# CIAM-Group/ComputerVision_Codes

Measured on AMD Instinct MI355X. Metric: frames/sec spatial-extract + per-video TCN latency, Cholec80, 1/2/4/8 GPU, higher is better.
Workload: dtype bf16

## Files before the change

### computervision_codes_amd/_lib.py

```python
from __future__ import annotations

import ctypes as C
import os

import torch

_HERE = os.path.dirname(os.path.abspath(__file__))
LIB_PATH = os.path.join(_HERE, "libmt4hip.so")

MT4_F32 = 0
MT4_BF16 = 1


class ConvDesc(C.Structure):
    _fields_ = [
        ("x", C.c_void_p), ("w", C.c_void_p), ("bias", C.c_void_p), ("residual", C.c_void_p), ("y", C.c_void_p),
        ("out_row_map", C.c_void_p),
        ("B", C.c_int32), ("H", C.c_int32), ("W", C.c_int32), ("Cin", C.c_int32),
        ("Ho", C.c_int32), ("Wo", C.c_int32), ("Cout", C.c_int32),
        ("KH", C.c_int32), ("KW", C.c_int32),
        ("stride_h", C.c_int32), ("stride_w", C.c_int32),
        ("pad_h", C.c_int32), ("pad_w", C.c_int32),
        ("dil_h", C.c_int32), ("dil_w", C.c_int32),
        ("relu", C.c_int32), ("dtype", C.c_int32), ("out_dtype", C.c_int32), ("tile", C.c_int32),
# ... 73 lines not shown
    "mt4_bn_stats_t": (C.c_int, [_vp, _i32, _vp, _vp, _vp, _vp, _vp, C.c_int64, _i32, C.c_float, C.c_float, _vp]),
    "mt4_avgpool1d_rows": (C.c_int, [_vp, _vp, _i32, _i32, _i32, _i32, _i32, _i32, _vp]),
    "mt4_interp_linear_rows": (C.c_int, [_vp, _vp, _i32, _i32, _i32, _i32, _i32, _vp]),
    "mt4_avgpool1d_rows_bwd_f32": (C.c_int, [_vp, _vp, _i32, _i32, _i32, _i32, _i32, _vp]),
    "mt4_interp_linear_rows_bwd_f32": (C.c_int, [_vp, _vp, _i32, _i32, _i32, _i32, _vp]),
    "mt4_bn_apply_sums_f32": (C.c_int, [_vp] * 10 + [C.c_int64, _i32, C.c_float, C.c_float, _i32, _vp]),
    "mt4_bn_apply_sums_t": (C.c_int, [_vp, _i32] + [_vp] * 9 + [C.c_int64, _i32, C.c_float, C.c_float, _i32, _vp]),
    "mt4_bn_apply_t": (C.c_int, [_vp, _i32, _vp, _vp, _vp, _vp, _vp, _vp, C.c_int64, _i32, _i32, _vp]),
    "mt4_bn_backward_t": (C.c_int, [_vp, _vp, _vp, _i32] + [_vp] * 9 + [C.c_int64, _i32, _i32, _vp]),
    "mt4_wgrad_conv2d_bf16": (C.c_int, [_vp, _vp, _vp] + [_i32] * 9 + [_vp]),
    "mt4_maxpool3x3s2_bwd_bf16": (C.c_int, [_vp, _vp, _vp, _i32, _i32, _i32, _i32, _vp]),
    "mt4_avgpool_bwd_bf16": (C.c_int, [_vp, _vp, _i32, _i32, _i32, _vp]),
    "mt4_cast_f32_bf16": (C.c_int, [_vp, _vp, C.c_int64, _vp]),
    "mt4_refresh_weights": (C.c_int, [_vp, _i32, C.c_int64, _vp]),
    "mt4_repack_weight_bf16": (C.c_int, [_vp, _vp, _i32, _i32, _i32, _i32, _vp]),
    "mt4_kd_mix_bwd_f32": (C.c_int, [_vp] * 9 + [_i32, _i32, _vp]),
    "mt4_tcn_conv": (C.c_int, [C.POINTER(TcnDesc), _vp]),
    "mt4_tcn_dilated_residual_layer": (C.c_int, [_vp] * 7 + [_i32] * 5 + [_vp]),
    "mt4_tcn_stage": (C.c_int, [_vp] * 5 + [C.POINTER(_vp)] * 4 + [_i32] * 5 + [_vp]),
    "mt4_bottleneck_packed_bytes": (C.c_int64, [_i32, _i32]),
    "mt4_bottleneck_pack_bf16": (C.c_int, [_vp] * 4 + [_i32, _vp, _vp]),
    "mt4_bottleneck_fused_bf16": (C.c_int, [_vp] * 7 + [_i32] * 5 + [_vp]),
    "mt4_pack_fragments_bf16": (C.c_int, [_vp, _i32, _i32, _vp, _vp]),
    "mt4_chain_gemm_bf16": (C.c_int, [_vp, C.c_int64, C.c_int64, _i32, _vp, _vp, _i32, _vp, _vp, _i32, _vp, _vp, _i32, _vp, _i32, _vp, _vp]),
    "mt4_bottleneck_next_packed_bytes": (C.c_int64, []),
    "mt4_bottleneck_pack_next_bf16": (C.c_int, [_vp, _vp, _vp]),
    "mt4_bottleneck_fused_next_bf16": (C.c_int, [_vp, _vp, _vp, _vp, _vp, _vp, _vp, _vp, _vp, _i32, _i32, _i32, _vp]),
    "mt4_fpn_topdown": (C.c_int, [_vp, _vp, _i32, C.c_int64, _i32, _vp]),
    "mt4_tcn_layer_fused_bf16": (C.c_int, [_vp, _vp, _vp, _vp, _vp, _vp, _i32, _i32, _i32, _i32, _vp]),
    "mt4_tcn_linear_ln_f32": (C.c_int, [_vp, _vp, _vp, _vp, _vp, _vp, _i32, _i32, _i32, C.c_float, _i32, _vp, _vp, _vp]),
    "mt4_tcn_linear_stats_f32": (C.c_int, [_vp, _vp, _vp, _vp, _vp, _i32, _i32, _i32, _i32, _vp, _vp]),
    "mt4_bgemm_f32": (C.c_int, [_vp, _vp, _vp, _i32, _i32, _i32, _i32, _i32, C.POINTER(C.c_int64), C.POINTER(C.c_int64), C.POINTER(C.c_int64),
                                C.c_float, _i32, _vp]),
    "mt4_softmax_rows_f32": (C.c_int, [_vp, C.c_int64, _i32, C.c_float, _vp]),
    "mt4_softmax_bwd_rows_f32": (C.c_int, [_vp, _vp, C.c_int64, _i32, C.c_float, _vp]),
    "mt4_layernorm_bwd_f32": (C.c_int, [_vp, _vp, _vp, _vp, _vp, _vp, C.c_int64, _i32, C.c_float, _i32, _vp]),
    "mt4_gelu_f32": (C.c_int, [_vp, _vp, C.c_int64, _vp]),
    "mt4_gelu_bwd_f32": (C.c_int, [_vp, _vp, _vp, C.c_int64, _vp]),
    "mt4_dwconv1d_k3_bwd_f32": (C.c_int, [_vp, _vp, _vp, _vp, _vp, _vp, _i32, _i32, _i32, _vp]),
    "mt4_gather_rows_f32": (C.c_int, [_vp, _vp, _vp, C.c_int64, _i32, _i32, _i32, _i32, _i32, _vp]),
    "mt4_add_bias_mask_f32": (C.c_int, [_vp, _vp, _vp, _vp, C.c_int64, _i32, _i32, _i32, _vp]),
    "mt4_relpos_table_grad_f32": (C.c_int, [_vp, _vp, _vp, C.c_int64, _i32, _i32, _vp]),
    "mt4_rowscale_add_f32": (C.c_int, [_vp, _vp, _vp, _vp, C.c_int64, _i32, _i32, _vp]),
    "mt4_groupwise_linear_bwd_f32": (C.c_int, [_vp] * 6 + [_i32, _i32, _i32, _vp]),
    "mt4_sum_over_batch_f32": (C.c_int, [_vp, _vp, _i32, C.c_int64, _i32, _vp]),
    "mt4_dropout_mask_f32": (C.c_int, [_vp, C.c_int64, C.c_int64, C.c_int64, C.c_float, _vp]),
    "mt4_axpby_f32": (C.c_int, [_vp, _vp, C.c_int64, C.c_float, C.c_float, _vp]),
# ... 49 lines not shown
```

### computervision_codes_amd/csrc/chain_gemm.hip

```cpp
#include "mt4_common.h"

typedef __bf16 bf16x8_t __attribute__((ext_vector_type(8)));

namespace {

struct ChainK {
    const char* x;
    long long x_ld_bytes;
    const char* w1f;
    const float* b1;
    const char* r1;
    char* y1;
    const char* w2f;
    const float* b2;
    const char* r2;
    char* y2;
    int M, K1, N1, N2, act1, act2;
};

constexpr int BM = 128;
constexpr int CH = 128;
constexpr int PLANE = BM * 128;

__device__ __forceinline__ void act4(float (&v)[4], int a) {
    if (a == 1) {
#pragma unroll
        for (int e = 0; e < 4; ++e) v[e] = fmaxf(v[e], 0.f);
    } else if (a == 2) {
        gelu_erf_n(v);
    }
}

template <int NT2, int NKS1, bool CONV, int NCHUNK>
__global__ __launch_bounds__(512, 2) void chain_gemm_kernel(const ChainK a) {
    extern __shared__ __attribute__((aligned(16))) char smem[];
    const int tid = threadIdx.x, lane = tid & 63;
    const int wave = __builtin_amdgcn_readfirstlane(tid >> 6);
    const int r16 = lane & 15, q = lane >> 4;
    const int m0 = blockIdx.x * BM;
    constexpr int nks1 = NKS1;
    constexpr int ACT1 = CONV ? 1 : 2;
    constexpr int nchunk = NCHUNK;
    const int mlast = a.M - 1;
    char* const Xs = smem;
    char* const Hb = smem + nks1 * PLANE;
    float* const B1s = (float*)(Hb + 4 * PLANE);
    const long long n1b = (long long)a.N1 * 2, n2b = (long long)a.N2 * 2;

    {
        uint4 xv[NKS1 * 2];
#pragma unroll
        for (int i = 0; i < NKS1 * 2; ++i) {
            const int pid = tid + i * 512;
            const int plane = pid >> 10, row = (pid >> 3) & 127, ck = pid & 7;
            xv[i] = *(const uint4*)(a.x + (long long)min(m0 + row, mlast) * a.x_ld_bytes + plane * 128 + ck * 16);
        }
#pragma unroll
        for (int i = 0; i < NKS1 * 2; ++i) {
            const int pid = tid + i * 512;
            const int plane = pid >> 10, row = (pid >> 3) & 127, ck = pid & 7;
            *(uint4*)(Xs + plane * PLANE + row * 128 + ((ck ^ (row & 7)) << 4)) = xv[i];
        }
    }
    struct R4 { uint4 v0, v1, v2, v3; };
    R4 rr;
    auto load_r = [&](int c) __attribute__((always_inline)) -> R4 {
        R4 r;
        const char* base = a.r1 + (long long)(c * CH) * 2;
        auto piece = [&](int i) __attribute__((always_inline)) -> uint4 {
            const int pid = tid + i * 512;
            const int plane = pid >> 10, row = (pid >> 3) & 127, ck = pid & 7;
            return *(const uint4*)(base + (long long)min(m0 + row, mlast) * n1b + plane * 128 + ck * 16);
        };
        r.v0 = piece(0); r.v1 = piece(1); r.v2 = piece(2); r.v3 = piece(3);
        return r;
    };
    auto put_r = [&](int c, const R4& r) __attribute__((always_inline)) {
        char* hb = Hb + (c & 1) * (2 * PLANE);
        auto dst = [&](int i) __attribute__((always_inline)) -> uint4* {
            const int pid = tid + i * 512;
            const int plane = pid >> 10, row = (pid >> 3) & 127, ck = pid & 7;
            return (uint4*)(hb + plane * PLANE + row * 128 + ((ck ^ (row & 7)) << 4));
        };
        *dst(0) = r.v0; *dst(1) = r.v1; *dst(2) = r.v2; *dst(3) = r.v3;
    };
    for (int i = tid; i < nchunk * (CH / 4); i += 512) *(float4*)(B1s + i * 4) = *(const float4*)(a.b1 + i * 4);
    if constexpr (CONV) {
        put_r(0, load_r(0));
        rr = load_r(min(1, nchunk - 1));
    }

    const int f1_stride = (a.K1 >> 5) * 1024;
    const int f2_stride = (a.N1 >> 5) * 1024;
    const char* const w1p = a.w1f + (long long)wave * f1_stride + lane * 16;
    const char* const w2p = a.w2f + (long long)(wave * NT2) * f2_stride + lane * 16;
    uint4 fa1[2 * NKS1];
    auto load_w1 = [&](int c) __attribute__((always_inline)) {
        const char* p = w1p + (long long)c * 8 * f1_stride;
#pragma unroll
        for (int s = 0; s < 2 * NKS1; ++s) fa1[s] = *(const uint4*)(p + s * 1024);
    };
    load_w1(0);

    f32x4 acc2[NT2][8];
#pragma unroll
    for (int t = 0; t < NT2; ++t) {
        const float4 b = *(const float4*)(a.b2 + (wave * NT2 + t) * 16 + q * 4);
#pragma unroll
        for (int j = 0; j < 8; ++j) acc2[t][j] = (f32x4){b.x, b.y, b.z, b.w};
    }
    __syncthreads();

    const int frag_off = r16 * 128;
    const int sw0 = ((0 * 4 + q) ^ (r16 & 7)) << 4, sw1 = ((1 * 4 + q) ^ (r16 & 7)) << 4;

#pragma unroll
    for (int c = 0; c < nchunk; ++c) {
        char* const hb = Hb + (c & 1) * (2 * PLANE);
        f32x4 acc1[8];
        {
            const float4 b = *(const float4*)(B1s + (c * 8 + wave) * 16 + q * 4);
#pragma unroll
            for (int j = 0; j < 8; ++j) acc1[j] = (f32x4){b.x, b.y, b.z, b.w};
        }
        uint4 fa2[NT2][4];
#pragma unroll
        for (int ks = 0; ks < NKS1; ++ks) {
            const char* xp = Xs + ks * PLANE + frag_off;
#pragma unroll
            for (int kk = 0; kk < 2; ++kk) {
                const bf16x8_t A = __builtin_bit_cast(bf16x8_t, fa1[ks * 2 + kk]);
#pragma unroll
                for (int jh = 0; jh < 8; jh += 4) {
                    uint4 bx[4];
#pragma unroll
                    for (int j = 0; j < 4; ++j) bx[j] = *(const uint4*)(xp + (jh + j) * (16 * 128) + (kk ? sw1 : sw0));
#pragma unroll
                    for (int j = 0; j < 4; ++j)
                        acc1[jh + j] = __builtin_amdgcn_mfma_f32_16x16x32_bf16(A, __builtin_bit_cast(bf16x8_t, bx[j]), acc1[jh + j], 0, 0, 0);
                }
                if (ks == 0 && kk == 0) {
#pragma unroll
                    for (int t = 0; t < NT2; ++t)
#pragma unroll
                        for (int s = 0; s < 4; ++s) fa2[t][s] = *(const uint4*)(w2p + (long long)t * f2_stride + (c * 4 + s) * 1024);
                }
            }
        }
        load_w1(min(c + 1, nchunk - 1));
        __syncthreads();
        {
            const int cl = wave * 16 + q * 4;
            const int plane = cl >> 6, cb = (cl & 63) * 2;
#pragma unroll
            for (int j = 0; j < 8; ++j) {
                const int row = j * 16 + r16;
                char* hp = hb + plane * PLANE + row * 128 + (((cb >> 4) ^ (row & 7)) << 4) + (cb & 8);
                float v[4] = {acc1[j][0], acc1[j][1], acc1[j][2], acc1[j][3]};
                if constexpr (CONV) {
                    const uint2 r = *(const uint2*)hp;
                    v[0] += __uint_as_float(r.x << 16); v[1] += __uint_as_float(r.x & 0xffff0000u);
                    v[2] += __uint_as_float(r.y << 16); v[3] += __uint_as_float(r.y & 0xffff0000u);
                }
                act4(v, ACT1);
                *(uint2*)hp = make_uint2(pack_bf16x2(v[0], v[1]), pack_bf16x2(v[2], v[3]));
            }
        }
        if constexpr (CONV) {
            put_r(c + 1, rr);
            rr = load_r(min(c + 2, nchunk - 1));
        }
        __syncthreads();
        if constexpr (CONV) {
#pragma unroll
            for (int i = 0; i < 4; ++i) {
                const int pid = tid + i * 512;
                const int plane = pid >> 10, row = (pid >> 3) & 127, ck = pid & 7;
                if (m0 + row < a.M)
                    *(uint4*)(a.y1 + (long long)(m0 + row) * n1b + (c * CH + plane * 64) * 2 + ck * 16) =
                        *(const uint4*)(hb + plane * PLANE + row * 128 + ((ck ^ (row & 7)) << 4));
            }
        }
#pragma unroll
        for (int p = 0; p < 2; ++p) {
            const char* hp = hb + p * PLANE + frag_off;
#pragma unroll
            for (int kk = 0; kk < 2; ++kk) {
                uint4 bx[8];
#pragma unroll
                for (int j = 0; j < 8; ++j) bx[j] = *(const uint4*)(hp + j * (16 * 128) + (kk ? sw1 : sw0));
#pragma unroll
                for (int t = 0; t < NT2; ++t) {
                    const bf16x8_t A = __builtin_bit_cast(bf16x8_t, fa2[t][p * 2 + kk]);
#pragma unroll
                    for (int j = 0; j < 8; ++j)
                        acc2[t][j] = __builtin_amdgcn_mfma_f32_16x16x32_bf16(A, __builtin_bit_cast(bf16x8_t, bx[j]), acc2[t][j], 0, 0, 0);
                }
            }
        }
    }
    __syncthreads();

    constexpr int ACT2 = CONV ? 1 : 0;
    const int pitch = a.N2 * 2 + 16;
    uint2 r2v[NT2][8];
    if constexpr (!CONV) {
#pragma unroll
        for (int t = 0; t < NT2; ++t)
#pragma unroll
            for (int j = 0; j < 8; ++j)
                r2v[t][j] = *(const uint2*)(a.r2 + (long long)min(m0 + j * 16 + r16, mlast) * n2b + ((wave * NT2 + t) * 16 + q * 4) * 2);
    }
#pragma unroll
    for (int t = 0; t < NT2; ++t) {
        const int n = (wave * NT2 + t) * 16 + q * 4;
#pragma unroll
        for (int j = 0; j < 8; ++j) {
            const int row = j * 16 + r16;
            float v[4] = {acc2[t][j][0], acc2[t][j][1], acc2[t][j][2], acc2[t][j][3]};
            if constexpr (!CONV) {
                const uint2 r = r2v[t][j];
                v[0] += __uint_as_float(r.x << 16); v[1] += __uint_as_float(r.x & 0xffff0000u);
                v[2] += __uint_as_float(r.y << 16); v[3] += __uint_as_float(r.y & 0xffff0000u);
            }
            act4(v, ACT2);
            *(uint2*)(smem + row * pitch + n * 2) = make_uint2(pack_bf16x2(v[0], v[1]), pack_bf16x2(v[2], v[3]));
        }
    }
    __syncthreads();
    const int vpr = a.N2 >> 3;
    for (int i = tid; i < BM * vpr; i += 512) {
        const int row = i / vpr, ck = i - row * vpr;
        if (m0 + row < a.M) *(uint4*)(a.y2 + (long long)(m0 + row) * n2b + ck * 16) = *(const uint4*)(smem + row * pitch + ck * 16);
    }
}

}

extern "C" int mt4_chain_gemm_bf16(const void* x, int64_t x_ld, int64_t M, int32_t K1, const void* w1_frag, const float* b1, int32_t N1, const void* r1,
                                   void* y1, int32_t act1, const void* w2_frag, const float* b2, int32_t N2, const void* r2, int32_t act2, void* y2,
                                   void* stream) {
    mt4_clear_error();
    if (!x || !w1_frag || !b1 || !w2_frag || !b2 || !y2 || M <= 0 || x_ld < K1) return MT4_EINVAL;
    if (K1 <= 0 || K1 > 256 || (K1 & 63) || N1 < 2 * CH || (N1 % CH) || (N2 != 128 && N2 != 256)) return MT4_EUNSUPPORTED;
    if (act1 < 0 || act1 > 2 || act2 < 0 || act2 > 2) return MT4_EINVAL;
    if ((((uintptr_t)x | (uintptr_t)w1_frag | (uintptr_t)w2_frag | (uintptr_t)r1 | (uintptr_t)y1 | (uintptr_t)r2 | (uintptr_t)y2 | (uintptr_t)b1 | (uintptr_t)b2) & 15) ||
        (x_ld & 7))
        return MT4_EALIGN;
    if (M > (int64_t)0x7fffffff - BM) return MT4_EUNSUPPORTED;
    ChainK k;
    k.x = (const char*)x; k.x_ld_bytes = x_ld * 2; k.w1f = (const char*)w1_frag; k.b1 = b1; k.r1 = (const char*)r1; k.y1 = (char*)y1;
    k.w2f = (const char*)w2_frag; k.b2 = b2; k.r2 = (const char*)r2; k.y2 = (char*)y2;
    k.M = (int)M; k.K1 = K1; k.N1 = N1; k.N2 = N2; k.act1 = act1; k.act2 = act2;
    const int xs = (K1 / 64) * PLANE;
    const int out = BM * (N2 * 2 + 16);
    const int lds = xs + 4 * PLANE + N1 * 4 > out ? xs + 4 * PLANE + N1 * 4 : out;
    const int grid = (int)((M + BM - 1) / BM);
    const bool conv = r1 != nullptr;
    if (conv != (y1 != nullptr) || act1 != (conv ? 1 : 2) || act2 != (conv ? 1 : 0) || conv == (r2 != nullptr)) return MT4_EUNSUPPORTED;
    if (K1 != 128 && K1 != 256) return MT4_EUNSUPPORTED;
#define MT4_CHAIN_LAUNCH(NT2_, NKS1_, CONV_, NCH_)                                                 \
    do {                                                                                       \
        auto fn = chain_gemm_kernel<NT2_, NKS1_, CONV_, NCH_>;                                 \
        MT4_RAISE_LDS(fn);                                                                     \
        hipLaunchKernelGGL(fn, dim3(grid), dim3(512), lds, (hipStream_t)stream, k);            \
    } while (0)
    const int nch = N1 / CH;
    if (nch != 4 && nch != 8) return MT4_EUNSUPPORTED;
    if (conv) {
        if (N2 == 256 && K1 == 256 && nch == 8) MT4_CHAIN_LAUNCH(2, 4, true, 8);
        else if (N2 == 256 && K1 == 128 && nch == 4) MT4_CHAIN_LAUNCH(2, 2, true, 4);
        else if (N2 == 128 && K1 == 128 && nch == 4) MT4_CHAIN_LAUNCH(1, 2, true, 4);
        else return MT4_EUNSUPPORTED;
    } else {
        if (N2 == 256 && K1 == 256 && nch == 8) MT4_CHAIN_LAUNCH(2, 4, false, 8);
        else if (N2 == 128 && K1 == 128 && nch == 4) MT4_CHAIN_LAUNCH(1, 2, false, 4);
        else return MT4_EUNSUPPORTED;
    }
#undef MT4_CHAIN_LAUNCH
    return mt4_check_launch();
// ... 2 lines not shown
```

### computervision_codes_amd/ops.py

```python
from __future__ import annotations

import contextlib
import contextvars
import os
import ctypes as C
import functools
from typing import Optional, Tuple

import torch

from . import _lib
from ._lib import MT4_BF16, MT4_F32, ConvDesc, check, lib

_DT = {torch.float32: MT4_F32, torch.bfloat16: MT4_BF16}


def _stream() -> int:
    return torch.cuda.current_stream().cuda_stream


def _need_cuda(*ts):
    for t in ts:
        if t is not None and not t.is_cuda:
            raise _lib.Mt4Error("mt4 ops need device tensors (no CPU fallback exists)")
# ... 131 lines not shown
    return out


def pack_fragments(w_packed: torch.Tensor) -> torch.Tensor:
    _need_cuda(w_packed)
    assert w_packed.dtype == torch.bfloat16 and w_packed.is_contiguous() and w_packed.dim() == 2
    out = torch.empty_like(w_packed)
    check(lib.mt4_pack_fragments_bf16(w_packed.data_ptr(), w_packed.shape[0], w_packed.shape[1], out.data_ptr(), _stream()), "mt4_pack_fragments_bf16")
    return out


def chain_gemm_supported(k1: int, n1: int, n2: int, conv: bool) -> bool:
    return (k1, n1, n2) in ((256, 1024, 256), (128, 512, 128)) or (conv and (k1, n1, n2) == (128, 512, 256))


CHAIN_MIN_TILES = 48


def chain_gemm_pays(rows: int) -> bool:
    return (rows + 127) // 128 >= CHAIN_MIN_TILES and not _LATENCY_TILES.get()


def chain_gemm(x2d: torch.Tensor, w1_frag: torch.Tensor, b1: torch.Tensor, w2_frag: torch.Tensor, b2: torch.Tensor, *, r1: Optional[torch.Tensor] = None,
               r2: Optional[torch.Tensor] = None, y1: Optional[torch.Tensor] = None, y2: Optional[torch.Tensor] = None):
    _need_cuda(x2d, w1_frag, b1, w2_frag, b2, r1, r2, y1, y2)
    assert x2d.dim() == 2 and x2d.dtype == torch.bfloat16 and x2d.stride(1) == 1 and (r1 is None) != (r2 is None)
    m, k1 = x2d.shape
    n1, n2 = w1_frag.shape[0], w2_frag.shape[0]
    assert tuple(w1_frag.shape) == (n1, k1) and tuple(w2_frag.shape) == (n2, n1) and w1_frag.dtype == w2_frag.dtype == torch.bfloat16
    assert b1.dtype == b2.dtype == torch.float32 and b1.numel() == n1 and b2.numel() == n2
    conv = r1 is not None
    if conv:
        assert r1.dtype == torch.bfloat16 and r1.is_contiguous() and r1.numel() == m * n1
        y1 = torch.empty((m, n1), dtype=torch.bfloat16, device=x2d.device) if y1 is None else y1
        assert y1.dtype == torch.bfloat16 and y1.is_contiguous() and y1.numel() == m * n1
    else:
        assert r2.dtype == torch.bfloat16 and r2.is_contiguous() and r2.numel() == m * n2 and y1 is None
    y2 = torch.empty((m, n2), dtype=torch.bfloat16, device=x2d.device) if y2 is None else y2
    assert y2.dtype == torch.bfloat16 and y2.is_contiguous() and y2.numel() == m * n2
    check(lib.mt4_chain_gemm_bf16(x2d.data_ptr(), x2d.stride(0), m, k1, w1_frag.data_ptr(), b1.data_ptr(), n1, r1.data_ptr() if conv else None,
                                  y1.data_ptr() if conv else None, 1 if conv else 2, w2_frag.data_ptr(), b2.data_ptr(), n2,
                                  None if conv else r2.data_ptr(), 1 if conv else 0, y2.data_ptr(), _stream()), "mt4_chain_gemm_bf16")
    return y1, y2


def conv3x3_expand(x: torch.Tensor, w2_packed: torch.Tensor, b2: torch.Tensor, w3_frag: torch.Tensor, b3: torch.Tensor, residual: torch.Tensor,
                   out: Optional[torch.Tensor] = None) -> Optional[torch.Tensor]:
    _need_cuda(x, w2_packed, b2, w3_frag, b3, residual, out)
    b, h, w_, cin = x.shape
    cout3 = w3_frag.shape[0]
    assert x.dtype == torch.bfloat16 and x.is_contiguous() and cin == 128 and tuple(w2_packed.shape) == (128, packed_k(128, 3, 3, torch.bfloat16))
    assert w3_frag.dtype == torch.bfloat16 and w3_frag.shape[1] == 128 and residual.is_contiguous() and tuple(residual.shape) == (b, h, w_, cout3)
    y = torch.empty((b, h, w_, cout3), dtype=torch.bfloat16, device=x.device) if out is None else out
    assert y.is_contiguous() and tuple(y.shape) == (b, h, w_, cout3) and y.dtype == torch.bfloat16
    d = ConvDesc(x.data_ptr(), w2_packed.data_ptr(), b2.data_ptr(), residual.data_ptr(), y.data_ptr(), None,
                 b, h, w_, cin, h, w_, 128, 3, 3, 1, 1, 1, 1, 1, 1, 1, dt_code(x.dtype), dt_code(x.dtype), 0, 0, 0, 0, 0, 0, cout3,
                 w3_frag.data_ptr(), b3.data_ptr(), y.data_ptr(), 1, 0, None, 0, 0, 0, 0, 1)
    rc = lib.mt4_conv_nhwc(C.byref(d), _stream())
    if rc == _lib.MT4_EUNSUPPORTED:
        return None
    check(rc, "mt4_conv_nhwc")
    return y


def tcn_conv(x: torch.Tensor, w_packed: torch.Tensor, bias: Optional[torch.Tensor], *, taps: int, dilation: int = 1,
# ... 955 lines not shown
```

### computervision_codes_amd/spatial_cnn.py

```python
from __future__ import annotations

from typing import Dict, Optional

import torch

from . import ops
from .shapes import resnet_feat_dim, spatial_cnn_shapes
from .synth import IMAGENET_MEAN, IMAGENET_STD

_DEPTHS = {"resnet18": (2, 2, 2, 2), "resnet50": (3, 4, 6, 3)}
_HEADS = (("i", 6), ("v", 10), ("t", 15), ("ivt", 100))


class VideoNas:

    def __init__(self, args=None, num_tool=6, num_verb=10, num_target=15, num_triplet=100, dtype: torch.dtype = torch.float32,
                 device: str = "cuda"):
        self.args = args
        self.network = args.network
        self.loss_type = args.loss_type
        self.feat_dim = getattr(args, "student_dim", None) or resnet_feat_dim(self.network)
        assert self.feat_dim == resnet_feat_dim(self.network), "student_dim must equal the trunk's feature width"
        self.dtype = dtype
        self.device = torch.device(device)
# ... 129 lines not shown
                    if bi == n - 1 and li < last and self.fuse_downsample and self.fuse_next_block and nq in self._p:
                        x, pending = ops.bottleneck_fused_next(x, self._p[q + "fused"], self._p[nq])
                        x_is_even = True
                    else:
                        x = ops.bottleneck_fused(x, self._p[q + "fused"], out=o_buf)
                    continue
                if bottleneck and (q + "conv3ds") in self._p and self.fuse_downsample:
                    o = self._conv(pending if pending is not None else self._conv(x, q + "conv1", 1), q + "conv2", 3, stride=s, pad=1)
                    pending = None
                    wcat, bcat = self._p[q + "conv3ds"]
                    x = ops.conv_nhwc(o, wcat, bcat, kh=1, kw=1, relu=True, out=o_buf, second=(x, 1 if x_is_even else s))
                    x_is_even = False
                    continue
                idt = self._conv(x, q + "ds", 1, stride=s, relu=False) if (q + "ds") in self._p else x
                if bottleneck:
                    o = pending if pending is not None else self._conv(x, q + "conv1", 1)
                    pending = None
                    nq = f"{pre}layer{li}.{bi + 1}." if bi + 1 < n else (f"{pre}layer{li + 1}.0." if li < last else None)
                    if (li in self.chain_layers and nq is not None and o_buf is None and self.dtype == torch.bfloat16 and (q + "conv3frag") in self._p
                            and (nq + "conv1frag") in self._p and ops.chain_gemm_pays(o.shape[0] * ((o.shape[1] - 1) // s + 1) * ((o.shape[2] - 1) // s + 1))
                            and ops.chain_gemm_supported(self._p[q + "conv3frag"].shape[1], self._p[q + "conv3frag"].shape[0], self._p[nq + "conv1frag"].shape[0], True)):
                        o = self._conv(o, q + "conv2", 3, stride=s, pad=1)
                        bb, hh, ww, cc = o.shape
                        y1, t1 = ops.chain_gemm(o.view(-1, cc), self._p[q + "conv3frag"], self._p[q + "conv3"][1], self._p[nq + "conv1frag"],
                                                self._p[nq + "conv1"][1], r1=idt)
                        x, pending = y1.view(bb, hh, ww, -1), t1.view(bb, hh, ww, -1)
                        continue
                    if (q + "conv3frag") in self._p and li == 2 and self.fuse_expand:
                        (w2, b2), b3 = self._p[q + "conv2"], self._p[q + "conv3"][1]
                        y = ops.conv3x3_expand(o, w2, b2, self._p[q + "conv3frag"], b3, idt, out=o_buf)
                        if y is not None:
                            x = y
                            continue
                    o = self._conv(o, q + "conv2", 3, stride=s, pad=1)
                    x = self._conv(o, q + "conv3", 1, residual=idt, out=o_buf)
                else:
                    o = self._conv(x, q + "conv1", 3, stride=s, pad=1)
                    x = self._conv(o, q + "conv2", 3, pad=1, residual=idt, out=o_buf)
        return x

    def trunk_from_padded(self, xp: torch.Tensor, h: int, w: int) -> torch.Tensor:
        return ops.global_avgpool(self._layers(self._stem(xp, h, w), 1, 4))

    def conv_plan(self, h: int, w: int):
        plan = []
        ho, wo = (h - 1) // 2 + 1, (w - 1) // 2 + 1
        plan.append(dict(name="stem", Cin=3, Cout=64, kh=7, kw=7, stride=2, Ho=ho, Wo=wo))
        hh, ww = (ho - 1) // 2 + 1, (wo - 1) // 2 + 1
        cin = 64
# ... 133 lines not shown
```

### include/mt4hip.h

```cpp
#ifndef MT4HIP_H
#define MT4HIP_H

#include <stddef.h>
#include <stdint.h>

#ifdef __cplusplus
extern "C" {
#endif

#define MT4_OK 0
#define MT4_EINVAL (-1)
#define MT4_EALIGN (-2)
#define MT4_ELAUNCH (-3)
#define MT4_EUNSUPPORTED (-4)

#define MT4_F32 0
#define MT4_BF16 1

int mt4_abi_version(void);
const char* mt4_source_digest(void);
const char* mt4_strerror(int code);
int mt4_last_hip_error(void);

#define MT4_STAT_REPLICAS 8
// ... 25 lines not shown
    void* fuse_y;
    int32_t fuse_relu;
    int32_t residual_float;
    const void* x2;
    int32_t x2_H, x2_W, x2_C;
    int32_t x2_stride;
    int32_t fuse_expand;
    double* stat_sums;
} mt4_conv_desc;

int mt4_conv_nhwc(const mt4_conv_desc* d, void* stream);
int mt4_conv_tile_count(void);

int64_t mt4_bottleneck_packed_bytes(int32_t Cin, int32_t has_downsample);
int mt4_bottleneck_pack_bf16(const void* w1, const void* w2, const void* w3, const void* wds, int32_t Cin, void* out, void* stream);
int mt4_bottleneck_fused_bf16(const void* x, void* y, const void* w_frag, const float* b1, const float* b2, const float* b3, const float* bds,
                              int32_t B, int32_t H, int32_t W, int32_t Cin, int32_t mid, void* stream);
int64_t mt4_bottleneck_next_packed_bytes(void);
int mt4_bottleneck_pack_next_bf16(const void* w1_next, void* out, void* stream);
int mt4_bottleneck_fused_next_bf16(const void* x, void* y_even, void* t_next, const void* w_frag, const float* b1, const float* b2, const float* b3,
                                   const void* w_next, const float* b_next, int32_t B, int32_t H, int32_t W, void* stream);
int mt4_pack_fragments_bf16(const void* w_packed, int32_t rows, int32_t row_elems, void* out, void* stream);
int mt4_chain_gemm_bf16(const void* x, int64_t x_ld, int64_t M, int32_t K1, const void* w1_frag, const float* b1, int32_t N1, const void* r1, void* y1,
                        int32_t act1, const void* w2_frag, const float* b2, int32_t N2, const void* r2, int32_t act2, void* y2, void* stream);
int64_t mt4_conv_packed_k(int32_t Cin, int32_t KH, int32_t KW, int32_t dtype);

int mt4_pack_conv_weight(const float* w_oihw, const float* scale, void* w_packed, int32_t Cout, int32_t Cin,
                         int32_t KH, int32_t KW, int32_t dtype, void* stream);

int mt4_pack_stem_weight(const float* w_oihw, const float* scale, void* w_packed, int32_t Cout, int32_t dtype,
                         void* stream);

int mt4_preprocess_u8(const uint8_t* frames, void* out, int32_t B, int32_t H, int32_t W, const float mean[3],
                      const float std[3], int32_t dtype, void* stream);
int mt4_pad_nchw_f32(const float* x, void* out, int32_t B, int32_t H, int32_t W, int32_t dtype, void* stream);
int mt4_preprocess_u8_s2d(const uint8_t* frames, void* out, int32_t B, int32_t H, int32_t W, const float mean[3], const float std[3],
                          void* stream);

int mt4_png_inflate(const uint8_t* streams, const int64_t* offsets, const int32_t* lengths, uint8_t* raw, int32_t B, int64_t raw_stride,
                    int64_t raw_len, int32_t* status, void* stream);
int mt4_png_unfilter_rgb8(const uint8_t* raw, uint8_t* out, int32_t B, int32_t H, int32_t W, int64_t raw_stride, int32_t* status, void* stream);
int mt4_copy_spans_u8(const uint8_t* src, uint8_t* dst, const int64_t* src_off, const int64_t* dst_off, const int32_t* len, int32_t n, void* stream);
int mt4_png_stat_files(const char* const* paths, int32_t n, int64_t* sizes, int32_t threads);
int mt4_png_read_files(const char* const* paths, const int64_t* sizes, const int64_t* file_off, int32_t n, uint8_t* dst, int32_t* width,
                       int32_t* height, int64_t* span_off, int32_t* span_len, int32_t* nspans, int32_t max_spans, int32_t* status, int32_t threads);

int mt4_resize_pass_u8(const void* in, void* out, const int32_t* bounds, const int32_t* coeffs, int32_t ksize, int32_t B, int32_t Hin,
// ... 158 lines not shown
```

Baseline: 96490.

## Make chain GEMM persistent with async LDS loads and strided y1 writes

```diff
diff --git a/computervision_codes_amd/_lib.py b/computervision_codes_amd/_lib.py
--- a/computervision_codes_amd/_lib.py
+++ b/computervision_codes_amd/_lib.py
@@ -119,7 +119,7 @@
     "mt4_bottleneck_pack_bf16": (C.c_int, [_vp] * 4 + [_i32, _vp, _vp]),
     "mt4_bottleneck_fused_bf16": (C.c_int, [_vp] * 7 + [_i32] * 5 + [_vp]),
     "mt4_pack_fragments_bf16": (C.c_int, [_vp, _i32, _i32, _vp, _vp]),
-    "mt4_chain_gemm_bf16": (C.c_int, [_vp, C.c_int64, C.c_int64, _i32, _vp, _vp, _i32, _vp, _vp, _i32, _vp, _vp, _i32, _vp, _i32, _vp, _vp]),
+    "mt4_chain_gemm_bf16": (C.c_int, [_vp, C.c_int64, C.c_int64, _i32, _vp, _vp, _i32, _vp, _vp, _i32, _vp, _vp, _i32, _vp, _i32, _vp, _i32, _i32, _vp]),
     "mt4_bottleneck_next_packed_bytes": (C.c_int64, []),
     "mt4_bottleneck_pack_next_bf16": (C.c_int, [_vp, _vp, _vp]),
     "mt4_bottleneck_fused_next_bf16": (C.c_int, [_vp, _vp, _vp, _vp, _vp, _vp, _vp, _vp, _vp, _i32, _i32, _i32, _vp]),
diff --git a/computervision_codes_amd/csrc/chain_gemm.hip b/computervision_codes_amd/csrc/chain_gemm.hip
--- a/computervision_codes_amd/csrc/chain_gemm.hip
+++ b/computervision_codes_amd/csrc/chain_gemm.hip
@@ -16,6 +16,8 @@
     const char* r2;
     char* y2;
     int M, K1, N1, N2, act1, act2;
+    int ntiles;
+    int even_h, even_w;
 };
 
 constexpr int BM = 128;
@@ -31,44 +33,73 @@
     }
 }
 
+typedef unsigned chain_v4u __attribute__((ext_vector_type(4)));
+
+__device__ __forceinline__ chain_v4u chain_srd(const void* p, unsigned bytes) {
+    const unsigned long long u = (unsigned long long)p;
+    chain_v4u r;
+    r.x = __builtin_amdgcn_readfirstlane((unsigned)u);
+    r.y = __builtin_amdgcn_readfirstlane((unsigned)(u >> 32) & 0xffffu);
+    r.z = __builtin_amdgcn_readfirstlane(bytes);
+    r.w = 0x00020000u;
+    return r;
+}
+
+__device__ __forceinline__ void chain_dma16(chain_v4u srd, unsigned voff, unsigned lds_addr) {
+    unsigned keep;
+    asm volatile("s_mov_b32 %0, m0\n\ts_mov_b32 m0, %3\n\ts_nop 0\n\tbuffer_load_dwordx4 %1, %2, 0 offen lds\n\ts_mov_b32 m0, %0"
+                 : "=&s"(keep) : "v"(voff), "s"(srd), "s"(lds_addr) : "memory");
+}
+
+__device__ __forceinline__ void wait_vm0() { __builtin_amdgcn_s_waitcnt(0x0f70); }
+
 template <int NT2, int NKS1, bool CONV, int NCHUNK>
 __global__ __launch_bounds__(512, 2) void chain_gemm_kernel(const ChainK a) {
     extern __shared__ __attribute__((aligned(16))) char smem[];
-    const int tid = threadIdx.x, lane = tid & 63;
+    int tid = threadIdx.x;
+    int lane = tid & 63, r16 = lane & 15, q = lane >> 4;
     const int wave = __builtin_amdgcn_readfirstlane(tid >> 6);
-    const int r16 = lane & 15, q = lane >> 4;
-    const int m0 = blockIdx.x * BM;
     constexpr int nks1 = NKS1;
     constexpr int ACT1 = CONV ? 1 : 2;
     constexpr int nchunk = NCHUNK;
+    constexpr int N2 = 128 * NT2;
+    constexpr int OPITCH = N2 * 2 + 16;
+    constexpr int HB = 4 * PLANE > BM * OPITCH ? 4 * PLANE : BM * OPITCH;
     const int mlast = a.M - 1;
     char* const Xs = smem;
     char* const Hb = smem + nks1 * PLANE;
-    float* const B1s = (float*)(Hb + 4 * PLANE);
-    const long long n1b = (long long)a.N1 * 2, n2b = (long long)a.N2 * 2;
-
+    float* const B1s = (float*)(Hb + HB);
+    float* const B2s = B1s + nchunk * CH;
+    constexpr long long n1b = nchunk * CH * 2, n2b = N2 * 2;
+
+    int tile = blockIdx.x;
     {
-        uint4 xv[NKS1 * 2];
+        const int nb = gridDim.x;
+        const int q8 = nb >> 3, r8 = nb & 7;
+        const int xcd = tile & 7, local = tile >> 3;
+        tile = (xcd < r8 ? xcd * (q8 + 1) : r8 * (q8 + 1) + (xcd - r8) * q8) + local;
+    }
+    const int step = gridDim.x;
+
+    const unsigned xs_lds = __builtin_amdgcn_readfirstlane((unsigned)(uintptr_t)(__attribute__((address_space(3))) char*)Xs) + wave * 1024;
+    auto load_x = [&](int m0) __attribute__((always_inline)) {
+        const int rmax = mlast - m0;
+        const chain_v4u srd = chain_srd(a.x + (long long)m0 * a.x_ld_bytes, (unsigned)min((long long)rmax * a.x_ld_bytes + a.K1 * 2, 0x7fffffffLL));
 #pragma unroll
         for (int i = 0; i < NKS1 * 2; ++i) {
             const int pid = tid + i * 512;
-            const int plane = pid >> 10, row = (pid >> 3) & 127, ck = pid & 7;
-            xv[i] = *(const uint4*)(a.x + (long long)min(m0 + row, mlast) * a.x_ld_bytes + plane * 128 + ck * 16);
-        }
-#pragma unroll
-        for (int i = 0; i < NKS1 * 2; ++i) {
-            const int pid = tid + i * 512;
-            const int plane = pid >> 10, row = (pid >> 3) & 127, ck = pid & 7;
-            *(uint4*)(Xs + plane * PLANE + row * 128 + ((ck ^ (row & 7)) << 4)) = xv[i];
-        }
-    }
+            const int plane = pid >> 10, row = (pid >> 3) & 127, ck = (pid & 7) ^ (row & 7);
+            chain_dma16(srd, (unsigned)(min(row, rmax) * a.x_ld_bytes) + plane * 128 + ck * 16, xs_lds + i * 8192);
+        }
+    };
     struct R4 { uint4 v0, v1, v2, v3; };
-    R4 rr;
-    auto load_r = [&](int c) __attribute__((always_inline)) -> R4 {
+    auto load_r = [&](int m0, int c) __attribute__((always_inline)) -> R4 {
         R4 r;
         const char* base = a.r1 + (long long)(c * CH) * 2;
+        int t = tid;
+        asm volatile("" : "+v"(t));
         auto piece = [&](int i) __attribute__((always_inline)) -> uint4 {
-            const int pid = tid + i * 512;
+            const int pid = t + i * 512;
             const int plane = pid >> 10, row = (pid >> 3) & 127, ck = pid & 7;
             return *(const uint4*)(base + (long long)min(m0 + row, mlast) * n1b + plane * 128 + ck * 16);
         };
@@ -77,23 +108,33 @@
     };
     auto put_r = [&](int c, const R4& r) __attribute__((always_inline)) {
         char* hb = Hb + (c & 1) * (2 * PLANE);
+        int t = tid;
+        asm volatile("" : "+v"(t));
         auto dst = [&](int i) __attribute__((always_inline)) -> uint4* {
-            const int pid = tid + i * 512;
+            const int pid = t + i * 512;
             const int plane = pid >> 10, row = (pid >> 3) & 127, ck = pid & 7;
             return (uint4*)(hb + plane * PLANE + row * 128 + ((ck ^ (row & 7)) << 4));
         };
         *dst(0) = r.v0; *dst(1) = r.v1; *dst(2) = r.v2; *dst(3) = r.v3;
     };
+    auto y1_row = [&](int m) __attribute__((always_inline)) -> int {
+        if (m >= a.M) return -1;
+        if (a.even_w == 0) return m;
+        const int t = m / a.even_w, w = m - t * a.even_w, b = t / a.even_h, h = t - b * a.even_h;
+        if ((h | w) & 1) return -1;
+        return (b * ((a.even_h + 1) >> 1) + (h >> 1)) * ((a.even_w + 1) >> 1) + (w >> 1);
+    };
+
     for (int i = tid; i < nchunk * (CH / 4); i += 512) *(float4*)(B1s + i * 4) = *(const float4*)(a.b1 + i * 4);
-    if constexpr (CONV) {
-        put_r(0, load_r(0));
-        rr = load_r(min(1, nchunk - 1));
-    }
+    if (tid < N2 / 4) *(float4*)(B2s + tid * 4) = *(const float4*)(a.b2 + tid * 4);
+    load_x(tile * BM);
+    R4 rr;
+    if constexpr (CONV) rr = load_r(tile * BM, 0);
 
     const int f1_stride = (a.K1 >> 5) * 1024;
     const int f2_stride = (a.N1 >> 5) * 1024;
-    const char* const w1p = a.w1f + (long long)wave * f1_stride + lane * 16;
-    const char* const w2p = a.w2f + (long long)(wave * NT2) * f2_stride + lane * 16;
+    const char* w1p = a.w1f + (long long)wave * f1_stride + lane * 16;
+    const char* w2p = a.w2f + (long long)(wave * NT2) * f2_stride + lane * 16;
     uint4 fa1[2 * NKS1];
     auto load_w1 = [&](int c) __attribute__((always_inline)) {
         const char* p = w1p + (long long)c * 8 * f1_stride;
@@ -101,137 +142,165 @@
         for (int s = 0; s < 2 * NKS1; ++s) fa1[s] = *(const uint4*)(p + s * 1024);
     };
     load_w1(0);
-
-    f32x4 acc2[NT2][8];
-#pragma unroll
-    for (int t = 0; t < NT2; ++t) {
-        const float4 b = *(const float4*)(a.b2 + (wave * NT2 + t) * 16 + q * 4);
-#pragma unroll
-        for (int j = 0; j < 8; ++j) acc2[t][j] = (f32x4){b.x, b.y, b.z, b.w};
-    }
-    __syncthreads();
-
-    const int frag_off = r16 * 128;
-    const int sw0 = ((0 * 4 + q) ^ (r16 & 7)) << 4, sw1 = ((1 * 4 + q) ^ (r16 & 7)) << 4;
-
-#pragma unroll
-    for (int c = 0; c < nchunk; ++c) {
-        char* const hb = Hb + (c & 1) * (2 * PLANE);
-        f32x4 acc1[8];
-        {
-            const float4 b = *(const float4*)(B1s + (c * 8 + wave) * 16 + q * 4);
-#pragma unroll
-            for (int j = 0; j < 8; ++j) acc1[j] = (f32x4){b.x, b.y, b.z, b.w};
-        }
-        uint4 fa2[NT2][4];
-#pragma unroll
-        for (int ks = 0; ks < NKS1; ++ks) {
-            const char* xp = Xs + ks * PLANE + frag_off;
-#pragma unroll
-            for (int kk = 0; kk < 2; ++kk) {
-                const bf16x8_t A = __builtin_bit_cast(bf16x8_t, fa1[ks * 2 + kk]);
-#pragma unroll
-                for (int jh = 0; jh < 8; jh += 4) {
-                    uint4 bx[4];
-#pragma unroll
-                    for (int j = 0; j < 4; ++j) bx[j] = *(const uint4*)(xp + (jh + j) * (16 * 128) + (kk ? sw1 : sw0));
-#pragma unroll
-                    for (int j = 0; j < 4; ++j)
-                        acc1[jh + j] = __builtin_amdgcn_mfma_f32_16x16x32_bf16(A, __builtin_bit_cast(bf16x8_t, bx[j]), acc1[jh + j], 0, 0, 0);
-                }
-                if (ks == 0 && kk == 0) {
-#pragma unroll
-                    for (int t = 0; t < NT2; ++t)
-#pragma unroll
-                        for (int s = 0; s < 4; ++s) fa2[t][s] = *(const uint4*)(w2p + (long long)t * f2_stride + (c * 4 + s) * 1024);
-                }
-            }
-        }
-        load_w1(min(c + 1, nchunk - 1));
+    wait_vm0();
+
+    for (;;) {
+        asm volatile("" : "+v"(tid));
+        lane = tid & 63; r16 = lane & 15; q = lane >> 4;
+        w1p = a.w1f + (long long)wave * f1_stride + lane * 16;
+        w2p = a.w2f + (long long)(wave * NT2) * f2_stride + lane * 16;
+        const int frag_off = r16 * 128;
+        const int sw0 = ((0 * 4 + q) ^ (r16 & 7)) << 4, sw1 = ((1 * 4 + q) ^ (r16 & 7)) << 4;
+        const int m0 = tile * BM;
+        const int next = tile + step;
+        const bool more = next < a.ntiles;
+        const int m0n = (more ? next : tile) * BM;
+        int ya = 0, yb = 0;
+        if constexpr (CONV) {
+            ya = y1_row(m0 + (tid >> 3));
+            yb = y1_row(m0 + (tid >> 3) + 64);
+        }
         __syncthreads();
-        {
-            const int cl = wave * 16 + q * 4;
-            const int plane = cl >> 6, cb = (cl & 63) * 2;
+        if constexpr (CONV) {
+            put_r(0, rr);
+            rr = load_r(m0, min(1, nchunk - 1));
+        }
+        f32x4 acc2[NT2][8];
+#pragma unroll
+        for (int t = 0; t < NT2; ++t) {
+            const float4 b = *(const float4*)(B2s + (wave * NT2 + t) * 16 + q * 4);
+#pragma unroll
+            for (int j = 0; j < 8; ++j) acc2[t][j] = (f32x4){b.x, b.y, b.z, b.w};
+        }
+
+#pragma unroll
+        for (int c = 0; c < nchunk; ++c) {
+            char* const hb = Hb + (c & 1) * (2 * PLANE);
+            f32x4 acc1[8];
+            {
+                const float4 b = *(const float4*)(B1s + (c * 8 + wave) * 16 + q * 4);
+#pragma unroll
+                for (int j = 0; j < 8; ++j) acc1[j] = (f32x4){b.x, b.y, b.z, b.w};
+            }
+            uint4 fa2[NT2][4];
+#pragma unroll
+            for (int ks = 0; ks < NKS1; ++ks) {
+                const char* xp = Xs + ks * PLANE + frag_off;
+#pragma unroll
+                for (int kk = 0; kk < 2; ++kk) {
+                    const bf16x8_t A = __builtin_bit_cast(bf16x8_t, fa1[ks * 2 + kk]);
+#pragma unroll
+                    for (int jh = 0; jh < 8; jh += 4) {
+                        uint4 bx[4];
+#pragma unroll
+                        for (int j = 0; j < 4; ++j) bx[j] = *(const uint4*)(xp + (jh + j) * (16 * 128) + (kk ? sw1 : sw0));
+#pragma unroll
+                        for (int j = 0; j < 4; ++j)
+                            acc1[jh + j] = __builtin_amdgcn_mfma_f32_16x16x32_bf16(A, __builtin_bit_cast(bf16x8_t, bx[j]), acc1[jh + j], 0, 0, 0);
+                    }
+                    if (ks == 0 && kk == 0) {
+#pragma unroll
+                        for (int t = 0; t < NT2; ++t)
+#pragma unroll
+                            for (int s = 0; s < 4; ++s) fa2[t][s] = *(const uint4*)(w2p + (long long)t * f2_stride + (c * 4 + s) * 1024);
+                    }
+                }
+            }
+            load_w1((c + 1) % nchunk);
+            __syncthreads();
+            if (c == nchunk - 1 && more) load_x(m0n);
+            {
+                const int cl = wave * 16 + q * 4;
+                const int plane = cl >> 6, cb = (cl & 63) * 2;
+#pragma unroll
+                for (int j = 0; j < 8; ++j) {
+                    const int row = j * 16 + r16;
+                    char* hp = hb + plane * PLANE + row * 128 + (((cb >> 4) ^ (row & 7)) << 4) + (cb & 8);
+                    float v[4] = {acc1[j][0], acc1[j][1], acc1[j][2], acc1[j][3]};
+                    if constexpr (CONV) {
+                        const uint2 r = *(const uint2*)hp;
+                        v[0] += __uint_as_float(r.x << 16); v[1] += __uint_as_float(r.x & 0xffff0000u);
+                        v[2] += __uint_as_float(r.y << 16); v[3] += __uint_as_float(r.y & 0xffff0000u);
+                    }
+                    act4(v, ACT1);
+                    *(uint2*)hp = make_uint2(pack_bf16x2(v[0], v[1]), pack_bf16x2(v[2], v[3]));
+                }
+            }
+            if constexpr (CONV) {
+                if (c + 1 < nchunk) put_r(c + 1, rr);
+                if (c + 2 < nchunk) rr = load_r(m0, c + 2);
+                else if (c + 2 == nchunk) rr = load_r(m0n, 0);
+            }
+            __syncthreads();
+            if constexpr (CONV) {
+                int t = tid;
+                asm volatile("" : "+v"(ya), "+v"(yb), "+v"(t));
+#pragma unroll
+                for (int i = 0; i < 4; ++i) {
+                    const int pid = t + i * 512;
+                    const int plane = pid >> 10, row = (pid >> 3) & 127, ck = pid & 7;
+                    const int yr = (i & 1) ? yb : ya;
+                    if (yr >= 0)
+                        *(uint4*)(a.y1 + (long long)yr * n1b + (c * CH + plane * 64) * 2 + ck * 16) =
+                            *(const uint4*)(hb + plane * PLANE + row * 128 + ((ck ^ (row & 7)) << 4));
+                }
+            }
+#pragma unroll
+            for (int p = 0; p < 2; ++p) {
+                const char* hp = hb + p * PLANE + frag_off;
+#pragma unroll
+                for (int kk = 0; kk < 2; ++kk) {
+                    uint4 bx[8];
+#pragma unroll
+                    for (int j = 0; j < 8; ++j) bx[j] = *(const uint4*)(hp + j * (16 * 128) + (kk ? sw1 : sw0));
+#pragma unroll
+                    for (int t = 0; t < NT2; ++t) {
+                        const bf16x8_t A = __builtin_bit_cast(bf16x8_t, fa2[t][p * 2 + kk]);
+#pragma unroll
+                        for (int j = 0; j < 8; ++j)
+                            acc2[t][j] = __builtin_amdgcn_mfma_f32_16x16x32_bf16(A, __builtin_bit_cast(bf16x8_t, bx[j]), acc2[t][j], 0, 0, 0);
+                    }
+                }
+            }
+        }
+        __syncthreads();
+
+        constexpr int ACT2 = CONV ? 1 : 0;
+        uint2 r2v[NT2][8];
+        if constexpr (!CONV) {
+#pragma unroll
+            for (int t = 0; t < NT2; ++t)
+#pragma unroll
+                for (int j = 0; j < 8; ++j)
+                    r2v[t][j] = *(const uint2*)(a.r2 + (long long)min(m0 + j * 16 + r16, mlast) * n2b + ((wave * NT2 + t) * 16 + q * 4) * 2);
+        }
+#pragma unroll
+        for (int t = 0; t < NT2; ++t) {
+            const int n = (wave * NT2 + t) * 16 + q * 4;
 #pragma unroll
             for (int j = 0; j < 8; ++j) {
                 const int row = j * 16 + r16;
-                char* hp = hb + plane * PLANE + row * 128 + (((cb >> 4) ^ (row & 7)) << 4) + (cb & 8);
-                float v[4] = {acc1[j][0], acc1[j][1], acc1[j][2], acc1[j][3]};
-                if constexpr (CONV) {
-                    const uint2 r = *(const uint2*)hp;
+                float v[4] = {acc2[t][j][0], acc2[t][j][1], acc2[t][j][2], acc2[t][j][3]};
+                if constexpr (!CONV) {
+                    const uint2 r = r2v[t][j];
                     v[0] += __uint_as_float(r.x << 16); v[1] += __uint_as_float(r.x & 0xffff0000u);
                     v[2] += __uint_as_float(r.y << 16); v[3] += __uint_as_float(r.y & 0xffff0000u);
                 }
-                act4(v, ACT1);
-                *(uint2*)hp = make_uint2(pack_bf16x2(v[0], v[1]), pack_bf16x2(v[2], v[3]));
-            }
-        }
-        if constexpr (CONV) {
-            put_r(c + 1, rr);
-            rr = load_r(min(c + 2, nchunk - 1));
-        }
+                act4(v, ACT2);
+                *(uint2*)(Hb + row * OPITCH + n * 2) = make_uint2(pack_bf16x2(v[0], v[1]), pack_bf16x2(v[2], v[3]));
+            }
+        }
+        wait_vm0();
         __syncthreads();
-        if constexpr (CONV) {
-#pragma unroll
-            for (int i = 0; i < 4; ++i) {
-                const int pid = tid + i * 512;
-                const int plane = pid >> 10, row = (pid >> 3) & 127, ck = pid & 7;
-                if (m0 + row < a.M)
-                    *(uint4*)(a.y1 + (long long)(m0 + row) * n1b + (c * CH + plane * 64) * 2 + ck * 16) =
-                        *(const uint4*)(hb + plane * PLANE + row * 128 + ((ck ^ (row & 7)) << 4));
-            }
-        }
-#pragma unroll
-        for (int p = 0; p < 2; ++p) {
-            const char* hp = hb + p * PLANE + frag_off;
-#pragma unroll
-            for (int kk = 0; kk < 2; ++kk) {
-                uint4 bx[8];
-#pragma unroll
-                for (int j = 0; j < 8; ++j) bx[j] = *(const uint4*)(hp + j * (16 * 128) + (kk ? sw1 : sw0));
-#pragma unroll
-                for (int t = 0; t < NT2; ++t) {
-                    const bf16x8_t A = __builtin_bit_cast(bf16x8_t, fa2[t][p * 2 + kk]);
-#pragma unroll
-                    for (int j = 0; j < 8; ++j)
-                        acc2[t][j] = __builtin_amdgcn_mfma_f32_16x16x32_bf16(A, __builtin_bit_cast(bf16x8_t, bx[j]), acc2[t][j], 0, 0, 0);
-                }
-            }
-        }
-    }
-    __syncthreads();
-
-    constexpr int ACT2 = CONV ? 1 : 0;
-    const int pitch = a.N2 * 2 + 16;
-    uint2 r2v[NT2][8];
-    if constexpr (!CONV) {
-#pragma unroll
-        for (int t = 0; t < NT2; ++t)
-#pragma unroll
-            for (int j = 0; j < 8; ++j)
-                r2v[t][j] = *(const uint2*)(a.r2 + (long long)min(m0 + j * 16 + r16, mlast) * n2b + ((wave * NT2 + t) * 16 + q * 4) * 2);
-    }
-#pragma unroll
-    for (int t = 0; t < NT2; ++t) {
-        const int n = (wave * NT2 + t) * 16 + q * 4;
-#pragma unroll
-        for (int j = 0; j < 8; ++j) {
-            const int row = j * 16 + r16;
-            float v[4] = {acc2[t][j][0], acc2[t][j][1], acc2[t][j][2], acc2[t][j][3]};
-            if constexpr (!CONV) {
-                const uint2 r = r2v[t][j];
-                v[0] += __uint_as_float(r.x << 16); v[1] += __uint_as_float(r.x & 0xffff0000u);
-                v[2] += __uint_as_float(r.y << 16); v[3] += __uint_as_float(r.y & 0xffff0000u);
-            }
-            act4(v, ACT2);
-            *(uint2*)(smem + row * pitch + n * 2) = make_uint2(pack_bf16x2(v[0], v[1]), pack_bf16x2(v[2], v[3]));
-        }
-    }
-    __syncthreads();
-    const int vpr = a.N2 >> 3;
-    for (int i = tid; i < BM * vpr; i += 512) {
-        const int row = i / vpr, ck = i - row * vpr;
-        if (m0 + row < a.M) *(uint4*)(a.y2 + (long long)(m0 + row) * n2b + ck * 16) = *(const uint4*)(smem + row * pitch + ck * 16);
+        constexpr int vpr = N2 / 8;
+#pragma unroll
+        for (int i = 0; i < BM * vpr / 512; ++i) {
+            const int idx = tid + i * 512;
+            const int row = idx / vpr, ck = idx - row * vpr;
+            if (m0 + row < a.M) *(uint4*)(a.y2 + (long long)(m0 + row) * n2b + ck * 16) = *(const uint4*)(Hb + row * OPITCH + ck * 16);
+        }
+        if (!more) break;
+        tile = next;
     }
 }
 
@@ -239,7 +308,7 @@
 
 extern "C" int mt4_chain_gemm_bf16(const void* x, int64_t x_ld, int64_t M, int32_t K1, const void* w1_frag, const float* b1, int32_t N1, const void* r1,
                                    void* y1, int32_t act1, const void* w2_frag, const float* b2, int32_t N2, const void* r2, int32_t act2, void* y2,
-                                   void* stream) {
+                                   int32_t y1_even_h, int32_t y1_even_w, void* stream) {
     mt4_clear_error();
     if (!x || !w1_frag || !b1 || !w2_frag || !b2 || !y2 || M <= 0 || x_ld < K1) return MT4_EINVAL;
     if (K1 <= 0 || K1 > 256 || (K1 & 63) || N1 < 2 * CH || (N1 % CH) || (N2 != 128 && N2 != 256)) return MT4_EUNSUPPORTED;
@@ -248,14 +317,31 @@
         (x_ld & 7))
         return MT4_EALIGN;
     if (M > (int64_t)0x7fffffff - BM) return MT4_EUNSUPPORTED;
+    if (y1_even_h < 0 || y1_even_w < 0 || (y1_even_h == 0) != (y1_even_w == 0)) return MT4_EINVAL;
+    if (y1_even_h > 0 && (!y1 || M % ((int64_t)y1_even_h * y1_even_w))) return MT4_EINVAL;
     ChainK k;
     k.x = (const char*)x; k.x_ld_bytes = x_ld * 2; k.w1f = (const char*)w1_frag; k.b1 = b1; k.r1 = (const char*)r1; k.y1 = (char*)y1;
     k.w2f = (const char*)w2_frag; k.b2 = b2; k.r2 = (const char*)r2; k.y2 = (char*)y2;
     k.M = (int)M; k.K1 = K1; k.N1 = N1; k.N2 = N2; k.act1 = act1; k.act2 = act2;
+    k.ntiles = (int)((M + BM - 1) / BM);
+    k.even_h = y1_even_h; k.even_w = y1_even_w;
     const int xs = (K1 / 64) * PLANE;
     const int out = BM * (N2 * 2 + 16);
-    const int lds = xs + 4 * PLANE + N1 * 4 > out ? xs + 4 * PLANE + N1 * 4 : out;
-    const int grid = (int)((M + BM - 1) / BM);
+    const int lds = xs + (4 * PLANE > out ? 4 * PLANE : out) + (N1 + N2) * 4;
+    static int cus[64] = {};
+    int dev = 0;
+    (void)hipGetDevice(&dev);
+    int ncu = dev >= 0 && dev < 64 ? cus[dev] : 0;
+    if (ncu <= 0) {
+        const hipError_t e = hipDeviceGetAttribute(&ncu, hipDeviceAttributeMultiprocessorCount, dev);
+        if (e != hipSuccess || ncu <= 0) {
+            g_mt4_last_hip_error = (int)e;
+            return MT4_ELAUNCH;
+        }
+        if (dev >= 0 && dev < 64) cus[dev] = ncu;
+    }
+    const int per_cu = (160 * 1024) / lds < 2 ? 1 : 2;
+    const int grid = k.ntiles < ncu * per_cu ? k.ntiles : ncu * per_cu;
     const bool conv = r1 != nullptr;
     if (conv != (y1 != nullptr) || act1 != (conv ? 1 : 2) || act2 != (conv ? 1 : 0) || conv == (r2 != nullptr)) return MT4_EUNSUPPORTED;
     if (K1 != 128 && K1 != 256) return MT4_EUNSUPPORTED;
diff --git a/computervision_codes_amd/ops.py b/computervision_codes_amd/ops.py
--- a/computervision_codes_amd/ops.py
+++ b/computervision_codes_amd/ops.py
@@ -177,7 +177,8 @@
 
 
 def chain_gemm(x2d: torch.Tensor, w1_frag: torch.Tensor, b1: torch.Tensor, w2_frag: torch.Tensor, b2: torch.Tensor, *, r1: Optional[torch.Tensor] = None,
-               r2: Optional[torch.Tensor] = None, y1: Optional[torch.Tensor] = None, y2: Optional[torch.Tensor] = None):
+               r2: Optional[torch.Tensor] = None, y1: Optional[torch.Tensor] = None, y2: Optional[torch.Tensor] = None,
+               y1_even: Optional[Tuple[int, int, int]] = None):
     _need_cuda(x2d, w1_frag, b1, w2_frag, b2, r1, r2, y1, y2)
     assert x2d.dim() == 2 and x2d.dtype == torch.bfloat16 and x2d.stride(1) == 1 and (r1 is None) != (r2 is None)
     m, k1 = x2d.shape
@@ -185,17 +186,23 @@
     assert tuple(w1_frag.shape) == (n1, k1) and tuple(w2_frag.shape) == (n2, n1) and w1_frag.dtype == w2_frag.dtype == torch.bfloat16
     assert b1.dtype == b2.dtype == torch.float32 and b1.numel() == n1 and b2.numel() == n2
     conv = r1 is not None
+    eh = ew = 0
     if conv:
         assert r1.dtype == torch.bfloat16 and r1.is_contiguous() and r1.numel() == m * n1
-        y1 = torch.empty((m, n1), dtype=torch.bfloat16, device=x2d.device) if y1 is None else y1
-        assert y1.dtype == torch.bfloat16 and y1.is_contiguous() and y1.numel() == m * n1
+        m1 = m
+        if y1_even is not None:
+            eb, eh, ew = (int(v) for v in y1_even)
+            assert eb > 0 and eh > 0 and ew > 0 and eb * eh * ew == m
+            m1 = eb * ((eh + 1) // 2) * ((ew + 1) // 2)
+        y1 = torch.empty((m1, n1), dtype=torch.bfloat16, device=x2d.device) if y1 is None else y1
+        assert y1.dtype == torch.bfloat16 and y1.is_contiguous() and y1.numel() == m1 * n1
     else:
-        assert r2.dtype == torch.bfloat16 and r2.is_contiguous() and r2.numel() == m * n2 and y1 is None
+        assert r2.dtype == torch.bfloat16 and r2.is_contiguous() and r2.numel() == m * n2 and y1 is None and y1_even is None
     y2 = torch.empty((m, n2), dtype=torch.bfloat16, device=x2d.device) if y2 is None else y2
     assert y2.dtype == torch.bfloat16 and y2.is_contiguous() and y2.numel() == m * n2
     check(lib.mt4_chain_gemm_bf16(x2d.data_ptr(), x2d.stride(0), m, k1, w1_frag.data_ptr(), b1.data_ptr(), n1, r1.data_ptr() if conv else None,
                                   y1.data_ptr() if conv else None, 1 if conv else 2, w2_frag.data_ptr(), b2.data_ptr(), n2,
-                                  None if conv else r2.data_ptr(), 1 if conv else 0, y2.data_ptr(), _stream()), "mt4_chain_gemm_bf16")
+                                  None if conv else r2.data_ptr(), 1 if conv else 0, y2.data_ptr(), eh, ew, _stream()), "mt4_chain_gemm_bf16")
     return y1, y2
 
 
diff --git a/computervision_codes_amd/spatial_cnn.py b/computervision_codes_amd/spatial_cnn.py
--- a/computervision_codes_amd/spatial_cnn.py
+++ b/computervision_codes_amd/spatial_cnn.py
@@ -175,9 +175,11 @@
                             and ops.chain_gemm_supported(self._p[q + "conv3frag"].shape[1], self._p[q + "conv3frag"].shape[0], self._p[nq + "conv1frag"].shape[0], True)):
                         o = self._conv(o, q + "conv2", 3, stride=s, pad=1)
                         bb, hh, ww, cc = o.shape
+                        even = bi == n - 1 and self.fuse_downsample and (nq + "conv3ds") in self._p
                         y1, t1 = ops.chain_gemm(o.view(-1, cc), self._p[q + "conv3frag"], self._p[q + "conv3"][1], self._p[nq + "conv1frag"],
-                                                self._p[nq + "conv1"][1], r1=idt)
-                        x, pending = y1.view(bb, hh, ww, -1), t1.view(bb, hh, ww, -1)
+                                                self._p[nq + "conv1"][1], r1=idt, y1_even=(bb, hh, ww) if even else None)
+                        x = y1.view(bb, (hh + 1) // 2, (ww + 1) // 2, -1) if even else y1.view(bb, hh, ww, -1)
+                        pending, x_is_even = t1.view(bb, hh, ww, -1), even
                         continue
                     if (q + "conv3frag") in self._p and li == 2 and self.fuse_expand:
                         (w2, b2), b3 = self._p[q + "conv2"], self._p[q + "conv3"][1]
diff --git a/include/mt4hip.h b/include/mt4hip.h
--- a/include/mt4hip.h
+++ b/include/mt4hip.h
@@ -71,7 +71,8 @@
                                    const void* w_next, const float* b_next, int32_t B, int32_t H, int32_t W, void* stream);
 int mt4_pack_fragments_bf16(const void* w_packed, int32_t rows, int32_t row_elems, void* out, void* stream);
 int mt4_chain_gemm_bf16(const void* x, int64_t x_ld, int64_t M, int32_t K1, const void* w1_frag, const float* b1, int32_t N1, const void* r1, void* y1,
-                        int32_t act1, const void* w2_frag, const float* b2, int32_t N2, const void* r2, int32_t act2, void* y2, void* stream);
+                        int32_t act1, const void* w2_frag, const float* b2, int32_t N2, const void* r2, int32_t act2, void* y2,
+                        int32_t y1_even_h, int32_t y1_even_w, void* stream);
 int64_t mt4_conv_packed_k(int32_t Cin, int32_t KH, int32_t KW, int32_t dtype);
 
 int mt4_pack_conv_weight(const float* w_oihw, const float* scale, void* w_packed, int32_t Cout, int32_t Cin,
```

After: 96600 (median of 6 runs). About the same (+0.1%).
